# hkust-vgd/scanobjectnn

Hardware: AMD Instinct MI355X
Metric: point-clouds/sec fwd+bwd at B×2048×3, 15-cls (higher is better)
Workload: dtype f32

## Files before the change

### scanobjectnn_amd/csrc/mlp.hip

```cpp
#include <stdlib.h>

#include "common.h"
#include <initializer_list>
#include <type_traits>

#ifndef PCOPS_MLP_PART
#define PCOPS_MLP_PART (-1)
#endif
#define PCOPS_PART(p_) (PCOPS_MLP_PART < 0 || PCOPS_MLP_PART == (p_))
#define PCOPS_HIDDEN __attribute__((visibility("hidden")))

#ifndef PCOPS_BF_RM
#define PCOPS_BF_RM 1
#endif

namespace pcops_mlp {

typedef float f32x16 __attribute__((ext_vector_type(16)));
typedef float f32x4 __attribute__((ext_vector_type(4)));
typedef __bf16 bf16x8 __attribute__((ext_vector_type(8)));

typedef __bf16 bf16x2 __attribute__((ext_vector_type(2)));
typedef float f32x2 __attribute__((ext_vector_type(2)));
__device__ __forceinline__ void split3_pair(float a, float b, bf16x2 &h, bf16x2 &m, bf16x2 &l) {
// ... 4433 lines not shown
        }
    }
}

__global__ __launch_bounds__(256) void pool_top_wsparse_kernel(long long G, int S, int C, int Kp,
                                                               const float *__restrict__ gout,
                                                               const float *__restrict__ ysel,
                                                               const unsigned char *__restrict__ arg,
                                                               const float *__restrict__ sc, const float *__restrict__ sh,
                                                               const float *__restrict__ p,
                                                               const float *__restrict__ Yprev,
                                                               const float *__restrict__ psc, const float *__restrict__ psh,
                                                               float *__restrict__ Ssp, float *__restrict__ cfsum) {
    constexpr int KR = 8, U = 8;
    __shared__ float red[4][64 * KR + 1];
    const int lane = threadIdx.x & 63, wave = threadIdx.x >> 6;
    const int c = blockIdx.x;
    const float scc = sc[c], shc = sh[c], pc = p[c];
    const int kr = (Kp + 63) / 64;
    float asc[KR], ash[KR], acc[KR];
#pragma unroll
    for (int i = 0; i < KR; ++i) {
        const int k = lane + 64 * i;
        asc[i] = (k < Kp && psc) ? psc[k] : 1.f;
        ash[i] = (k < Kp && psc) ? psh[k] : 0.f;
        acc[i] = 0.f;
    }
    float csum = 0.f;
    const long long gq = (G + 3) / 4;
    const long long gend = (wave + 1) * gq < G ? (wave + 1) * gq : G;
    for (long long g0 = wave * gq; g0 < gend; g0 += 64) {
        const long long g = g0 + lane;
        float cf = 0.f;
        int row = 0;
        if (g < gend) {
            const long long e = g * C + c;
            cf = fmaf(ysel[e], scc, shc) > 0.f ? pc * gout[e] : 0.f;
            row = arg[e];
        }
        unsigned long long hits = __ballot(cf != 0.f);
        while (hits) {
            float w[U];
            long long r[U];
#pragma unroll
            for (int u = 0; u < U; ++u) {
                w[u] = 0.f;
                r[u] = 0;
                if (hits) {
                    const int l = __builtin_ctzll(hits);
                    hits &= hits - 1;
                    w[u] = __builtin_bit_cast(float, __builtin_amdgcn_readlane(__builtin_bit_cast(int, cf), l));
                    r[u] = (g0 + l) * S + __builtin_amdgcn_readlane(row, l);
                }
            }
#pragma unroll
            for (int i = 0; i < KR; ++i) {
                if (i >= kr) break;
                const int k = lane + 64 * i;
                float x[U];
#pragma unroll
                for (int u = 0; u < U; ++u) x[u] = (k < Kp) ? Yprev[r[u] * Kp + k] : 0.f;
#pragma unroll
                for (int u = 0; u < U; ++u) {
                    const float xv = psc ? fmaxf(fmaf(x[u], asc[i], ash[i]), 0.f) : x[u];
                    acc[i] = fmaf(w[u], xv, acc[i]);
                }
            }
#pragma unroll
            for (int u = 0; u < U; ++u) csum += w[u];
        }
    }
#pragma unroll
    for (int i = 0; i < KR; ++i) red[wave][lane + 64 * i] = acc[i];
    if (lane == 0) red[wave][64 * KR] = csum;
    __syncthreads();
    for (int k = threadIdx.x; k < Kp; k += 256)
        Ssp[(long long)k * C + c] = (red[0][k] + red[1][k]) + (red[2][k] + red[3][k]);
    if (threadIdx.x == 0)
        cfsum[c] = (red[0][64 * KR] + red[1][64 * KR]) + (red[2][64 * KR] + red[3][64 * KR]);
}

template <int KP>
__global__ __launch_bounds__(1024) void pool_top_addend_rows_kernel(int G, int C, const float *__restrict__ gout,
                                                                    const float *__restrict__ ysel,
                                                                    const unsigned char *__restrict__ arg,
                                                                    const float *__restrict__ sc, const float *__restrict__ sh,
                                                                    const float *__restrict__ p, const float *__restrict__ Wt,
                                                                    const int *__restrict__ block_start,
                                                                    float *__restrict__ addend, int *__restrict__ rowmap) {
    constexpr int LPR = KP / 4, RPP = 256 / LPR;
    constexpr int MAXR = 128, MW = 8;
    extern __shared__ __attribute__((aligned(16))) float lds[];
    float *Ws = lds;
    float *cf = Ws + (size_t)C * KP;
    unsigned *mask = reinterpret_cast<unsigned *>(cf + 4 * 256);
    const int tid = threadIdx.x, sub = tid >> 8, c = tid & 255;
    for (int e = tid; e < C * (KP / 4); e += 1024)
        reinterpret_cast<float4 *>(Ws)[e] = reinterpret_cast<const float4 *>(Wt)[e];
    const float scc = c < C ? sc[c] : 0.f, shc = c < C ? sh[c] : 0.f, pc = c < C ? p[c] : 0.f;
    float *mycf = cf + sub * 256;
    unsigned *mymask = mask + sub * MAXR * MW;
    const int q = c % LPR, rsub = c / LPR;
    float v = 0.f;
    int row = 0, base = 0, nrows = 0;
    auto fetch = [&](long long g) {
        v = 0.f; row = 0; base = 0; nrows = 0;
        if (g < G) {
            const int b0 = block_start[g];
            base = kBlk * b0;
            nrows = kBlk * (block_start[g + 1] - b0);
            nrows = nrows < MAXR ? nrows : MAXR;
            if (c < C) {
                const long long e = g * C + c;
                v = fmaf(ysel[e], scc, shc) > 0.f ? pc * gout[e] : 0.f;
                row = arg[e];
            }
        }
    };
    fetch((long long)blockIdx.x * 4 + sub);
    for (long long g0 = (long long)blockIdx.x * 4; g0 < G; g0 += (long long)gridDim.x * 4) {
        const float cv = v;
        const int crow = row, cbase = base, cnrows = nrows;
        __syncthreads();
        mycf[c] = cv;
#pragma unroll
        for (int i = 0; i < MAXR * MW / 256; ++i) mymask[c + 256 * i] = 0u;
        __syncthreads();
        if (cv != 0.f && crow < cnrows) atomicOr(&mymask[crow * MW + (c >> 5)], 1u << (c & 31));
        __syncthreads();
        fetch(g0 + (long long)gridDim.x * 4 + sub);
        for (int r = rsub; r < cnrows; r += RPP) {
            float4 acc = make_float4(0.f, 0.f, 0.f, 0.f);
            bool any = false;
#pragma unroll
            for (int w = 0; w < MW; ++w) {
                unsigned mm = mymask[r * MW + w];
                any = any || mm != 0u;
                while (mm) {
                    const int ch = 32 * w + __builtin_ctz(mm);
                    mm &= mm - 1u;
                    const float cw = mycf[ch];
                    const float4 wt = *reinterpret_cast<const float4 *>(&Ws[ch * KP + 4 * q]);
                    acc.x = fmaf(cw, wt.x, acc.x); acc.y = fmaf(cw, wt.y, acc.y);
                    acc.z = fmaf(cw, wt.z, acc.z); acc.w = fmaf(cw, wt.w, acc.w);
                }
            }
            const long long ri = (long long)cbase + r;
            if (any) *reinterpret_cast<float4 *>(&addend[ri * KP + 4 * q]) = acc;
            if (q == 0) rowmap[ri] = any ? (int)ri : -1;
        }
    }
}

template <int KP>
__global__ __launch_bounds__(256) void pool_top_wsparse_rows_kernel(int G, int C, int maxr, const float *__restrict__ gout,
                                                                    const float *__restrict__ ysel,
                                                                    const unsigned char *__restrict__ arg,
                                                                    const float *__restrict__ sc, const float *__restrict__ sh,
                                                                    const float *__restrict__ p,
                                                                    const float *__restrict__ Yprev,
                                                                    const float *__restrict__ psc, const float *__restrict__ psh,
                                                                    const int *__restrict__ block_start,
                                                                    float *__restrict__ part, float *__restrict__ part2) {
    constexpr int LD = KP + 1, K4 = KP / 4;
    extern __shared__ __attribute__((aligned(16))) float lds[];
    float *Xs = lds;
    const int tid = threadIdx.x, c = tid;
    const float scc = c < C ? sc[c] : 0.f, shc = c < C ? sh[c] : 0.f, pc = c < C ? p[c] : 0.f;
    const int k4 = tid % K4, r0 = tid / K4;
    const float4 asc = *reinterpret_cast<const float4 *>(psc + 4 * k4), ash = *reinterpret_cast<const float4 *>(psh + 4 * k4);
    float acc[KP];
#pragma unroll
    for (int k = 0; k < KP; ++k) acc[k] = 0.f;
    float csum = 0.f;
    for (int g = blockIdx.x; g < G; g += gridDim.x) {
        const int b0 = block_start[g];
        int nrows = kBlk * (block_start[g + 1] - b0);
        nrows = nrows < maxr ? nrows : maxr;
        const float *src = Yprev + (long long)kBlk * b0 * KP;
        float cfv = 0.f;
        int row = 0;
        if (c < C) {
            const long long e = (long long)g * C + c;
            cfv = fmaf(ysel[e], scc, shc) > 0.f ? pc * gout[e] : 0.f;
            row = arg[e];
            if (row >= nrows) { row = 0; cfv = 0.f; }
        }
        __syncthreads();
        for (int r = r0; r < nrows; r += 256 / K4) {
            float4 x = *reinterpret_cast<const float4 *>(src + (long long)r * KP + 4 * k4);
            x.x = fmaxf(fmaf(x.x, asc.x, ash.x), 0.f); x.y = fmaxf(fmaf(x.y, asc.y, ash.y), 0.f);
            x.z = fmaxf(fmaf(x.z, asc.z, ash.z), 0.f); x.w = fmaxf(fmaf(x.w, asc.w, ash.w), 0.f);
            float *d = &Xs[r * LD + 4 * k4];
            d[0] = x.x; d[1] = x.y; d[2] = x.z; d[3] = x.w;
        }
        __syncthreads();
        const float *xr = &Xs[row * LD];
#pragma unroll
        for (int k = 0; k < KP; ++k) acc[k] = fmaf(cfv, xr[k], acc[k]);
        csum += cfv;
    }
    if (c < C) {
        float *dst = part + (long long)blockIdx.x * KP * C + c;
#pragma unroll
        for (int k = 0; k < KP; ++k) dst[(long long)k * C] = acc[k];
        part2[(long long)blockIdx.x * C + c] = csum;
    }
}

template <int KP, int NR>
__global__ __launch_bounds__(256) void pool_top_wsparse_rows_pipe_kernel(int G, int C, int maxr, const float *__restrict__ gout,
                                                                         const float *__restrict__ ysel,
                                                                         const unsigned char *__restrict__ arg,
                                                                         const float *__restrict__ sc, const float *__restrict__ sh,
                                                                         const float *__restrict__ p,
                                                                         const float *__restrict__ Yprev,
                                                                         const float *__restrict__ psc, const float *__restrict__ psh,
                                                                         const int *__restrict__ block_start,
                                                                         float *__restrict__ part, float *__restrict__ part2) {
    constexpr int LD = KP + 4, K4 = KP / 4, RPP = 256 / K4;
    static_assert(NR * RPP == 64 || NR * RPP == 128, "the launcher sizes an LDS image at 64 or 128 rows (maxr <= NR RPP)");
    extern __shared__ __attribute__((aligned(16))) float lds[];
    const int tid = threadIdx.x, c = tid;
    const float scc = c < C ? sc[c] : 0.f, shc = c < C ? sh[c] : 0.f, pc = c < C ? p[c] : 0.f;
    const int k4 = tid % K4, r0 = tid / K4;
    const float4 asc = *reinterpret_cast<const float4 *>(psc + 4 * k4), ash = *reinterpret_cast<const float4 *>(psh + 4 * k4);
    float acc[KP];
#pragma unroll
    for (int k = 0; k < KP; ++k) acc[k] = 0.f;
    float csum = 0.f;
    const int grid = gridDim.x;
    float4 px[NR];
    float fy = 0.f, fg = 0.f;
    int fa = 0, fn = 0;
    int nb0 = 0, nb1 = 0;
    auto pair = [&](int g) {
        if (g < G) { nb0 = block_start[g]; nb1 = block_start[g + 1]; }
    };
    auto fetch = [&](int g) {
        const int n = g < G ? kBlk * (nb1 - nb0) : 0;
        fn = n < maxr ? n : maxr;
        const __amdgpu_buffer_rsrc_t rx = make_rsrc(Yprev + (long long)kBlk * (g < G ? nb0 : 0) * KP, (long long)fn * KP * 4);
#pragma unroll
        for (int j = 0; j < NR; ++j) px[j] = buf_load4(rx, (unsigned)((r0 + RPP * j) * KP + 4 * k4) * 4u, 0u);
        const long long e = (long long)(g < G ? g : G - 1) * C + (c < C ? c : C - 1);
        fy = ysel[e]; fg = gout[e]; fa = arg[e];
    };
    int g = blockIdx.x;
    pair(g);
    fetch(g);
    pair(g + grid);
    int buf = 0;
    for (; g < G; g += grid) {
        float *Xs = lds + buf * (NR * RPP * LD);
        int t0 = 0, t1 = 0;
        if (g + 2 * grid < G) {
            t0 = block_start[g + 2 * grid];
            t1 = block_start[g + 2 * grid + 1];
        }
#pragma unroll
        for (int j = 0; j < NR; ++j) {
            const int r = r0 + RPP * j;
            float4 x = px[j];
            x.x = fmaxf(fmaf(x.x, asc.x, ash.x), 0.f); x.y = fmaxf(fmaf(x.y, asc.y, ash.y), 0.f);
            x.z = fmaxf(fmaf(x.z, asc.z, ash.z), 0.f); x.w = fmaxf(fmaf(x.w, asc.w, ash.w), 0.f);
            *reinterpret_cast<float4 *>(&Xs[r * LD + 4 * k4]) = x;
        }
        float cfv = fmaf(fy, scc, shc) > 0.f ? pc * fg : 0.f;
        int row = fa;
        if (row >= fn || c >= C) { row = 0; cfv = 0.f; }
        fetch(g + grid);
        nb0 = t0; nb1 = t1;
        __syncthreads();
        const float *xr = &Xs[row * LD];
#pragma unroll
        for (int q = 0; q < K4; ++q) {
            const float4 v = *reinterpret_cast<const float4 *>(xr + 4 * q);
            acc[4 * q] = fmaf(cfv, v.x, acc[4 * q]); acc[4 * q + 1] = fmaf(cfv, v.y, acc[4 * q + 1]);
            acc[4 * q + 2] = fmaf(cfv, v.z, acc[4 * q + 2]); acc[4 * q + 3] = fmaf(cfv, v.w, acc[4 * q + 3]);
        }
        csum += cfv;
        buf ^= 1;
    }
    if (c < C) {
        float *dst = part + (long long)blockIdx.x * KP * C + c;
#pragma unroll
        for (int k = 0; k < KP; ++k) dst[(long long)k * C] = acc[k];
        part2[(long long)blockIdx.x * C + c] = csum;
    }
}

__device__ __forceinline__ void small_gemm_tile(int bx, int by, int M, int K, int N, const float *__restrict__ A, int lda,
                                                         const float *__restrict__ B, int ldb, float *__restrict__ C,
                                                         int ldc, int transA, int transB, const float *__restrict__ bias,
                                                         float *__restrict__ colsum) {
    __shared__ float As[4][32][17], Bs[4][16][33], red[4][32][33], cs[4][2][32];
    const int tid = threadIdx.x, lane = tid & 63, wave = tid >> 6;
    const int m0 = by * 32, n0 = bx * 32;
    const int kchunks = (K + 15) / 16;
    f32x16 acc;
#pragma unroll
    for (int v = 0; v < 16; ++v) acc[v] = 0.f;
    float ra[8], rb[8];
    auto fetch = [&](int ch) {
        const int k0 = ch * 16;
#pragma unroll
// ... 923 lines not shown
    const int groups = bwd_fused_groups(M, K, N, S, gpool != nullptr);
    if (const int rc = bwd_fused_args(a, M >= 1 && K >= 4 && K % 4 == 0 && N >= 1, groups, {xyzw, xyz_stats}, M, K, N, off4,
                                      a_scale, a_shift, G, Y, p, q, t, gpool, argmax, S, W, partial, dW, nullptr, stats_partial))
        return rc;
    a.amode = A_XYZ; a.ldx = 4; a.off4 = off4; a.xw = xyzw; a.xw_ld = K; a.xstats = xyz_stats;
    if (const int rc = set_rows(a, rows)) return rc;
    return bwd_fused_launch(a, true, groups, partial, dW, db, as_stream(stream));
}

int pcops_mlp_wgrad(long long M, int K, int N, const float *X, int ldx, const float *a_scale,
                    const float *a_shift, const float *G, const float *Y, const float *p, const float *q,
                    const float *t, const float *gpool, const unsigned char *argmax, int S,
                    const float *pool_scale, const float *pool_shift, float *partial, float *dW, float *db,
                    pcops_stream_t stream) {
    return pcops_mlp_wgrad_rows(M, K, N, X, ldx, a_scale, a_shift, G, Y, p, q, t, gpool, argmax, S, pool_scale,
                                pool_shift, partial, dW, db, nullptr, stream);
}

int pcops_mlp_wgrad_rows(long long M, int K, int N, const float *X, int ldx, const float *a_scale,
                         const float *a_shift, const float *G, const float *Y, const float *p, const float *q,
                         const float *t, const float *gpool, const unsigned char *argmax, int S,
                         const float *pool_scale, const float *pool_shift, float *partial, float *dW, float *db,
                         const pcops_rows_t *rows, pcops_stream_t stream) {
    PCOPS_REQUIRE_SHAPE(M >= 1 && K >= 1 && N >= 1 && ldx >= K);
    PCOPS_REQUIRE_PTR(X); PCOPS_REQUIRE_PTR(Y); PCOPS_REQUIRE_PTR(p); PCOPS_REQUIRE_PTR(q); PCOPS_REQUIRE_PTR(t);
    PCOPS_REQUIRE_PTR(partial); PCOPS_REQUIRE_PTR(dW);
    if (!gpool) PCOPS_REQUIRE_PTR(G);
    WgradArgs a = {};
    a.M = M; a.K = K; a.N = N;
    a.amode = a_scale ? A_BNRELU : A_PLAIN; a.X = X; a.ldx = ldx; a.asc = a_scale; a.ash = a_shift;
    a.dmode = gpool ? A_DYPOOL : A_DY; a.G = G; a.Y = Y; a.ldy = N; a.p = p; a.q = q; a.t = t;
    a.dsc = pool_scale; a.dsh = pool_shift; a.gpool = gpool; a.argmax = argmax; a.S = S > 0 ? S : 1;
    if (const int rc = set_rows(a, rows)) return rc;
    return wgrad_impl(a, partial, dW, db, as_stream(stream));
}

int pcops_mlp_wgrad_xyz(long long M, int K, int N, const float *off4, const float *xyzw, const float *a_scale,
                        const float *a_shift, const float *G, const float *Y, const float *p, const float *q,
                        const float *t, const float *gpool, const unsigned char *argmax, int S,
                        const float *pool_scale, const float *pool_shift, float *partial, float *dW, float *db,
                        pcops_stream_t stream) {
    return pcops_mlp_wgrad_xyz_rows(M, K, N, off4, xyzw, a_scale, a_shift, G, Y, p, q, t, gpool, argmax, S, pool_scale,
                                    pool_shift, partial, dW, db, nullptr, stream);
}

int pcops_mlp_wgrad_xyz_rows(long long M, int K, int N, const float *off4, const float *xyzw, const float *a_scale,
                             const float *a_shift, const float *G, const float *Y, const float *p, const float *q,
                             const float *t, const float *gpool, const unsigned char *argmax, int S,
                             const float *pool_scale, const float *pool_shift, float *partial, float *dW, float *db,
                             const pcops_rows_t *rows, pcops_stream_t stream) {
    PCOPS_REQUIRE_SHAPE(M >= 1 && K >= 1 && N >= 1);
    PCOPS_REQUIRE_PTR(off4); PCOPS_REQUIRE_PTR(xyzw); PCOPS_REQUIRE_PTR(a_scale); PCOPS_REQUIRE_PTR(a_shift);
    PCOPS_REQUIRE_PTR(Y); PCOPS_REQUIRE_PTR(p); PCOPS_REQUIRE_PTR(q); PCOPS_REQUIRE_PTR(t);
    PCOPS_REQUIRE_PTR(partial); PCOPS_REQUIRE_PTR(dW);
    if (!gpool) PCOPS_REQUIRE_PTR(G);
    if (reinterpret_cast<uintptr_t>(off4) & 15) return PCOPS_ERR_UNSUPPORTED;
    WgradArgs a = {};
    a.M = M; a.K = K; a.N = N;
    a.amode = A_XYZ; a.X = nullptr; a.ldx = K; a.asc = a_scale; a.ash = a_shift;
    a.off4 = off4; a.xw = xyzw; a.xw_ld = K;
    a.dmode = gpool ? A_DYPOOL : A_DY; a.G = G; a.Y = Y; a.ldy = N; a.p = p; a.q = q; a.t = t;
    a.dsc = pool_scale; a.dsh = pool_shift; a.gpool = gpool; a.argmax = argmax; a.S = S > 0 ? S : 1;
    if (const int rc = set_rows(a, rows)) return rc;
    return wgrad_impl(a, partial, dW, db, as_stream(stream));
}

static bool dgrad_top_plan(int M, int Kp, WsPlan *pl) {
    GemmArgs a = {};
    a.M = M; a.K = Kp; a.N = Kp; a.ldx = Kp; a.ldy = Kp;
    return ws_enabled() && Kp % 64 == 0 && Kp <= 512 && ws_plan(a, A_BNRELU, pl);
}

int pcops_mlp_pool_top_supported(int M, int Kp, int N, int S) {
    WsPlan pl;
    if (S < 1 || S > 256 || M % S != 0 || N % 4 != 0 || N > 1024) return 0;
    if (!dgrad_top_plan(M, Kp, &pl)) return 0;
    if (!(wgrad_pc_enabled() && wgrad_pc_shape_ok(M, Kp, Kp, Kp, true))) return 0;
    const long long slots = (long long)(M / S) * (S < N ? S : N);
    return slots * Kp * 4 < (long long)kOOB ? 1 : 0;
}

int pcops_mlp_pool_top_addend(int M, int Kp, int N, int S, const float *gout, const float *ysel,
                            const unsigned char *argmax, const float *pool_scale, const float *pool_shift,
                            const float *p, const float *Wt, float *addend, int *rowmap, pcops_stream_t stream) {
    PCOPS_REQUIRE_SHAPE(M >= 1 && S >= 1 && S <= 256 && M % S == 0 && Kp % 4 == 0 && N >= 1 && N <= 65535);
    PCOPS_REQUIRE_PTR(gout); PCOPS_REQUIRE_PTR(ysel); PCOPS_REQUIRE_PTR(argmax); PCOPS_REQUIRE_PTR(pool_scale);
    PCOPS_REQUIRE_PTR(pool_shift); PCOPS_REQUIRE_PTR(p); PCOPS_REQUIRE_PTR(Wt); PCOPS_REQUIRE_PTR(addend);
    PCOPS_REQUIRE_PTR(rowmap);
    if (reinterpret_cast<uintptr_t>(Wt) & 15 || reinterpret_cast<uintptr_t>(addend) & 15) return PCOPS_ERR_UNSUPPORTED;
    if (N > 1024 || Kp > 512) return PCOPS_ERR_UNSUPPORTED;
    if (M / S <= 512)
        hipLaunchKernelGGL(pool_top_addend_kernel<1024>, dim3(M / S), dim3(1024), 0, as_stream(stream), S, N, Kp,
                           S < N ? S : N, gout, ysel, argmax, pool_scale, pool_shift, p, Wt, addend, rowmap);
    else
        hipLaunchKernelGGL(pool_top_addend_kernel<256>, dim3(M / S), dim3(256), 0, as_stream(stream), S, N, Kp,
                           S < N ? S : N, gout, ysel, argmax, pool_scale, pool_shift, p, Wt, addend, rowmap);
    return pcops_launch_status();
}

int pcops_mlp_gemm_dgrad_top(int M, int Kp, const float *Yprev, const float *prev_scale, const float *prev_shift,
                             const float *Mq, const float *vconst, const float *addend, long long addend_rows,
                             const int *rowmap, float *Gprev, float *stats_partial, pcops_stream_t stream) {
    return pcops_mlp_gemm_dgrad_top_rows(M, Kp, Yprev, prev_scale, prev_shift, Mq, vconst, addend, addend_rows, rowmap, Gprev,
                                         stats_partial, nullptr, stream);
}

static int gram_finish(const GramArgs &g, int gg, float *gram, float *xsum, hipStream_t st) {
    const long long L = (long long)g.K * g.K;
    hipLaunchKernelGGL(sum_partials2_kernel, dim3(cdiv(L, 64) + (xsum ? cdiv(g.K, 64) : 0)), dim3(1024), 0, st, gg, L,
                       g.part, gram, (long long)g.K, g.xpart, xsum);
    hipLaunchKernelGGL(mirror_lower_kernel, dim3(g.K), dim3(256), 0, st, g.K, gram);
    return pcops_launch_status();
}

int pcops_mlp_gram(long long M, int Kp, const float *Yprev, int ldx, const float *a_scale, const float *a_shift,
                   float *partial, float *gram, float *xsum, pcops_stream_t stream) {
    PCOPS_REQUIRE_SHAPE(M >= 1 && Kp >= 1 && ldx >= Kp);
    PCOPS_REQUIRE_PTR(Yprev); PCOPS_REQUIRE_PTR(partial); PCOPS_REQUIRE_PTR(gram);
    PCOPS_REQUIRE_ARG((a_scale == nullptr) == (a_shift == nullptr));
    const int gg = gram_full_groups(M, Kp, ldx, Yprev);
    pcops_note_pipe(0);
    if (gg > 0) {
        hipStream_t st = as_stream(stream);
        GramArgs g = {M, Kp, ldx, Yprev, a_scale, a_shift, partial, partial + (long long)gg * Kp * Kp};
        const int nbk = (Kp + 31) / 32;
        const size_t lds = (size_t)(2 * 32 * nbk + 2 * 32 * (32 * nbk + 4)) * sizeof(float);
        const int rc = gram_full_launch(g, nbk, a_scale != nullptr, gg, lds, st);
        return rc ? rc : gram_finish(g, gg, gram, xsum, st);
    }
    WgradArgs a = {};
    a.M = M; a.K = Kp; a.N = Kp;
    a.amode = a_scale ? A_BNRELU : A_PLAIN; a.X = Yprev; a.ldx = ldx; a.asc = a_scale; a.ash = a_shift;
    a.dmode = A_SELFD; a.G = Yprev; a.Y = Yprev; a.ldy = ldx; a.p = a_scale; a.q = a_scale; a.t = a_shift; a.S = 1;
    return wgrad_impl(a, partial, gram, xsum, as_stream(stream));
}

int pcops_mlp_pool_top_wsparse(int M, int Kp, int N, int S, const float *gout, const float *ysel,
                               const unsigned char *argmax, const float *pool_scale, const float *pool_shift,
                               const float *p, const float *Yprev, const float *prev_scale, const float *prev_shift,
                               float *Ssp, float *cfsum, pcops_stream_t stream) {
    PCOPS_REQUIRE_SHAPE(M >= 1 && S >= 1 && S <= 256 && M % S == 0 && Kp >= 1 && Kp <= 512 && N >= 1);
    PCOPS_REQUIRE_PTR(gout); PCOPS_REQUIRE_PTR(ysel); PCOPS_REQUIRE_PTR(argmax); PCOPS_REQUIRE_PTR(pool_scale);
    PCOPS_REQUIRE_PTR(pool_shift); PCOPS_REQUIRE_PTR(p); PCOPS_REQUIRE_PTR(Yprev);
    PCOPS_REQUIRE_ARG((prev_scale == nullptr) == (prev_shift == nullptr));
    PCOPS_REQUIRE_PTR(Ssp); PCOPS_REQUIRE_PTR(cfsum);
    hipLaunchKernelGGL(pool_top_wsparse_kernel, dim3(N), dim3(256), 0, as_stream(stream), (long long)(M / S), S, N,
                       Kp, gout, ysel, argmax, pool_scale, pool_shift, p, Yprev, prev_scale, prev_shift, Ssp, cfsum);
    return pcops_launch_status();
}


static const int kTopRowsWs = 512;

int pcops_mlp_pool_top_rows_supported(int M, int Kp, int N, int S) {
    if (!pcops_mlp_pool_top_supported(M, Kp, N, S)) return 0;
    if (M < 65536 || S % kBlk != 0 || S > 128 || (Kp != 64 && Kp != 128) || N > 256 || N % 32 != 0) return 0;
    if (!gram_full_groups(M, Kp, Kp, nullptr)) return 0;
    return (long long)M * Kp * 4 < (long long)kOOB ? 1 : 0;
}

unsigned long long pcops_mlp_pool_top_wsparse_rows_partial(int Kp, int N) {
    return (unsigned long long)kTopRowsWs * ((unsigned long long)Kp * N + N);
}

int pcops_mlp_pool_top_addend_rows(int M, int Kp, int N, int S, const float *gout, const float *ysel,
                                   const unsigned char *argmax, const float *pool_scale, const float *pool_shift,
                                   const float *p, const float *Wt, float *addend, int *rowmap, const pcops_rows_t *rows,
                                   pcops_stream_t stream) {
    if (!rows) return pcops_mlp_pool_top_addend(M, Kp, N, S, gout, ysel, argmax, pool_scale, pool_shift, p, Wt, addend, rowmap, stream);
    PCOPS_REQUIRE_SHAPE(M >= 1 && S >= 1 && M % S == 0);
    PCOPS_REQUIRE_PTR(gout); PCOPS_REQUIRE_PTR(ysel); PCOPS_REQUIRE_PTR(argmax); PCOPS_REQUIRE_PTR(pool_scale);
    PCOPS_REQUIRE_PTR(pool_shift); PCOPS_REQUIRE_PTR(p); PCOPS_REQUIRE_PTR(Wt); PCOPS_REQUIRE_PTR(addend);
    PCOPS_REQUIRE_PTR(rowmap);
    { const int rrc = rows_ok(rows); if (rrc) return rrc; }
    if (!pcops_mlp_pool_top_rows_supported(M, Kp, N, S)) return PCOPS_ERR_UNSUPPORTED;
    if (reinterpret_cast<uintptr_t>(Wt) & 15 || reinterpret_cast<uintptr_t>(addend) & 15) return PCOPS_ERR_UNSUPPORTED;
    const int G = M / S;
    const size_t lds = ((size_t)N * Kp + 4 * 256 + 4 * 128 * 8) * sizeof(float);
    const int grid = (G + 3) / 4 < 256 ? (G + 3) / 4 : 256;
    hipStream_t st = as_stream(stream);
    return pcops_dispatch<64, 128>(Kp, PCOPS_ERR_UNSUPPORTED, [&](auto kp_) {
        return pcops_launch_lds(pool_top_addend_rows_kernel<decltype(kp_)::value>, dim3(grid), dim3(1024), lds, 160 * 1024, st, G, N,
                                gout, ysel, argmax, pool_scale, pool_shift, p, Wt, rows->block_start, addend, rowmap);
    });
}

int pcops_mlp_pool_top_wsparse_rows(int M, int Kp, int N, int S, const float *gout, const float *ysel,
                                    const unsigned char *argmax, const float *pool_scale, const float *pool_shift,
                                    const float *p, const float *Yprev, const float *prev_scale, const float *prev_shift,
                                    float *Ssp, float *cfsum, float *partial, const pcops_rows_t *rows,
                                    pcops_stream_t stream) {
    if (!rows) return pcops_mlp_pool_top_wsparse(M, Kp, N, S, gout, ysel, argmax, pool_scale, pool_shift, p, Yprev, prev_scale, prev_shift, Ssp, cfsum, stream);
    PCOPS_REQUIRE_SHAPE(M >= 1 && S >= 1 && M % S == 0);
    PCOPS_REQUIRE_PTR(gout); PCOPS_REQUIRE_PTR(ysel); PCOPS_REQUIRE_PTR(argmax); PCOPS_REQUIRE_PTR(pool_scale);
    PCOPS_REQUIRE_PTR(pool_shift); PCOPS_REQUIRE_PTR(p); PCOPS_REQUIRE_PTR(Yprev); PCOPS_REQUIRE_PTR(prev_scale);
    PCOPS_REQUIRE_PTR(prev_shift); PCOPS_REQUIRE_PTR(Ssp); PCOPS_REQUIRE_PTR(cfsum); PCOPS_REQUIRE_PTR(partial);
    { const int rrc = rows_ok(rows); if (rrc) return rrc; }
    if (!pcops_mlp_pool_top_rows_supported(M, Kp, N, S)) return PCOPS_ERR_UNSUPPORTED;
    if (reinterpret_cast<uintptr_t>(Yprev) & 15 || reinterpret_cast<uintptr_t>(prev_scale) & 15 ||
        reinterpret_cast<uintptr_t>(prev_shift) & 15)
        return PCOPS_ERR_UNSUPPORTED;
    const int G = M / S;
    const int grid = G < kTopRowsWs ? G : kTopRowsWs;
    const size_t lds = (size_t)S * (Kp + 1) * sizeof(float);
    float *part2 = partial + (long long)kTopRowsWs * Kp * N;
    hipStream_t st = as_stream(stream);
    const int img_rows = S <= 64 ? 64 : 128;
    if (S > img_rows) return PCOPS_ERR_UNSUPPORTED;
    const size_t lds_pipe = (size_t)2 * img_rows * (Kp + 4) * sizeof(float);
    const bool piped = pcops_get_option(PCOPS_OPT_POOL_TOP_ROWS_PIPELINED) != 0;
    const int rc = pcops_dispatch<64, 128>(Kp, PCOPS_ERR_UNSUPPORTED, [&](auto kp_) {
        constexpr int KP = decltype(kp_)::value;
        auto kern = !piped ? pool_top_wsparse_rows_kernel<KP>
                  : S <= 64 ? pool_top_wsparse_rows_pipe_kernel<KP, KP / 16> : pool_top_wsparse_rows_pipe_kernel<KP, KP / 8>;
        return pcops_launch_lds(kern, dim3(grid), dim3(256), piped ? lds_pipe : lds, 160 * 1024, st, G, N, S, gout, ysel, argmax,
                                pool_scale, pool_shift, p, Yprev, prev_scale, prev_shift, rows->block_start, partial, part2);
    });
    if (rc) return rc;
    const long long L = (long long)Kp * N;
    hipLaunchKernelGGL(sum_partials2_kernel, dim3(cdiv(L, 64) + cdiv(N, 64)), dim3(1024), 0, st, grid, L, partial, Ssp,
                       (long long)N, part2, cfsum);
    return pcops_launch_status();
}

int pcops_mlp_gemm_dgrad_top_rows(int M, int Kp, const float *Yprev, const float *prev_scale, const float *prev_shift,
                                  const float *Mq, const float *vconst, const float *addend, long long addend_rows,
                                  const int *rowmap, float *Gprev, float *stats_partial, const pcops_rows_t *rows,
                                  pcops_stream_t stream) {
    PCOPS_REQUIRE_SHAPE(M >= 1 && Kp >= 1);
    PCOPS_REQUIRE_PTR(Yprev); PCOPS_REQUIRE_PTR(Mq);
    PCOPS_REQUIRE_PTR(vconst); PCOPS_REQUIRE_PTR(addend); PCOPS_REQUIRE_PTR(rowmap); PCOPS_REQUIRE_PTR(Gprev);
    PCOPS_REQUIRE_ARG((prev_scale == nullptr) == (prev_shift == nullptr));
    WsPlan pl;
    if (!dgrad_top_plan(M, Kp, &pl)) return PCOPS_ERR_UNSUPPORTED;
    GemmArgs a = {};
    a.M = M; a.K = Kp; a.N = Kp; a.X = Yprev; a.ldx = Kp; a.v0 = prev_scale; a.v1 = prev_shift;
    a.W = Mq; a.Y = Gprev; a.ldy = Kp; a.Yprev = Yprev; a.msc = prev_scale; a.msh = prev_shift;
    a.stats = stats_partial; a.addend = addend; a.rowmap = rowmap; a.add_ld = Kp; a.vconst = vconst;
    a.add_bytes = addend_rows * Kp * 4;
    if (addend_rows < 1 || a.add_bytes >= (long long)kOOB) return PCOPS_ERR_UNSUPPORTED;
    if (const int rc = set_rows(a, rows)) return rc;
    if (!prev_scale) {
        a.stats = nullptr;
        return launch_gemm_ws_only<A_PLAIN, E_PLAINA>(a, as_stream(stream));
    }
    return launch_gemm_ws_only<A_BNRELU, E_MASKA>(a, as_stream(stream));
}

int pcops_mlp_gram_rows(long long M, int Kp, const float *Yprev, int ldx, const float *a_scale, const float *a_shift,
                        float *partial, float *gram, float *xsum, const pcops_rows_t *rows, pcops_stream_t stream) {
    if (!rows) return pcops_mlp_gram(M, Kp, Yprev, ldx, a_scale, a_shift, partial, gram, xsum, stream);
    PCOPS_REQUIRE_SHAPE(M >= 1 && Kp >= 1 && ldx >= Kp);
    PCOPS_REQUIRE_PTR(Yprev); PCOPS_REQUIRE_PTR(partial); PCOPS_REQUIRE_PTR(gram); PCOPS_REQUIRE_PTR(a_scale);
    PCOPS_REQUIRE_PTR(a_shift);
    { const int rrc = rows_ok(rows); if (rrc) return rrc; }
    const int gg = gram_full_groups(M, Kp, ldx, Yprev);
    if (gg <= 0 || (Kp != 64 && Kp != 128)) return PCOPS_ERR_UNSUPPORTED;
    pcops_note_pipe(0);
    hipStream_t st = as_stream(stream);
    GramArgs g = {M, Kp, ldx, Yprev, a_scale, a_shift, partial, partial + (long long)gg * Kp * Kp,
                  static_cast<const RowBlock *>(rows->blocks), rows->rows};
    const int nbk = Kp / 32;
    const size_t lds = (size_t)(2 * 32 * nbk + 2 * 32 * (32 * nbk + 4)) * sizeof(float);
    const bool bf3 = Kp == 128 && pcops_get_option(PCOPS_OPT_GRAM_SPLIT_BF16) != 0;
    const int rc = bf3 ? gram_rows_bf3_launch(g, gg, st) : gram_full_rows_launch(g, nbk, gg, lds, st);
    if (rc) return rc;
    if (bf3) pcops_note_pipe(1);
    return gram_finish(g, gg, gram, xsum, st);
}

int pcops_mlp_dy_apply(long long M, int N, const float *G, const float *Y, const float *p, const float *q, const float *t,
                       float *out, pcops_stream_t stream) {
    PCOPS_REQUIRE_SHAPE(M >= 0 && N >= 4 && N % 4 == 0);
    if (M == 0) return PCOPS_OK;
    PCOPS_REQUIRE_PTR(G); PCOPS_REQUIRE_PTR(Y); PCOPS_REQUIRE_PTR(p); PCOPS_REQUIRE_PTR(q); PCOPS_REQUIRE_PTR(t); PCOPS_REQUIRE_PTR(out);
    PCOPS_REQUIRE_ARG(((uintptr_t)G | (uintptr_t)Y | (uintptr_t)p | (uintptr_t)q | (uintptr_t)t | (uintptr_t)out) % 16 == 0);
    const long long total4 = M * (N / 4);
    const unsigned grid = (unsigned)(cdiv(total4, 256) < 8192 ? cdiv(total4, 256) : 8192);
    hipLaunchKernelGGL(dy_apply_kernel, dim3(grid), dim3(256), 0, as_stream(stream), total4, N / 4,
                       reinterpret_cast<const float4 *>(G), reinterpret_cast<const float4 *>(Y),
                       reinterpret_cast<const float4 *>(p), reinterpret_cast<const float4 *>(q),
                       reinterpret_cast<const float4 *>(t), reinterpret_cast<float4 *>(out));
    return pcops_launch_status();
}

int pcops_mlp_pool_top_prep(int Kp, int N, const float *W, const float *b, const float *q, const float *t, float *Wt,
                            float *Wq, float *u, float *v, pcops_stream_t stream) {
    PCOPS_REQUIRE_SHAPE(Kp >= 1 && N >= 1);
    PCOPS_REQUIRE_PTR(W); PCOPS_REQUIRE_PTR(b); PCOPS_REQUIRE_PTR(q); PCOPS_REQUIRE_PTR(t);
    PCOPS_REQUIRE_PTR(Wt); PCOPS_REQUIRE_PTR(Wq); PCOPS_REQUIRE_PTR(u);
    const int gx = (N + 31) / 32;
    hipLaunchKernelGGL(pool_top_prep_kernel, dim3(gx, (Kp + 31) / 32 + (v ? ((Kp + 7) / 8 + gx - 1) / gx : 0)), dim3(256), 0,
                       as_stream(stream), Kp, N, W, b, q, t, Wt, Wq, u, v);
    return pcops_launch_status();
}

int pcops_mlp_pool_top_finish(int Kp, int N, long long M, float *dW, const float *Ssp, const float *xsum, const float *u,
                              const float *cfsum, const float *q, const float *W, const float *b, const float *t,
                              float *db, pcops_stream_t stream) {
    PCOPS_REQUIRE_SHAPE(Kp >= 1 && N >= 1 && M >= 1);
    PCOPS_REQUIRE_PTR(dW); PCOPS_REQUIRE_PTR(Ssp); PCOPS_REQUIRE_PTR(xsum); PCOPS_REQUIRE_PTR(u); PCOPS_REQUIRE_PTR(cfsum);
    PCOPS_REQUIRE_PTR(q); PCOPS_REQUIRE_PTR(W); PCOPS_REQUIRE_PTR(b); PCOPS_REQUIRE_PTR(t); PCOPS_REQUIRE_PTR(db);
    hipLaunchKernelGGL(pool_top_finish_kernel, dim3((N + 255) / 256, 8 + (Kp + 7) / 8), dim3(256), 0, as_stream(stream), Kp, N,
                       (float)M, dW, Ssp, xsum, u, cfsum, q, W, b, t, db);
    return pcops_launch_status();
}

int pcops_small_gemm(int M, int K, int N, const float *A, int lda, const float *B, int ldb, float *C, int ldc,
                     pcops_stream_t stream) {
    return pcops_small_gemm_ex(M, K, N, A, lda, 0, B, ldb, 0, nullptr, C, ldc, stream);
}

int pcops_small_gemm_ex(int M, int K, int N, const float *A, int lda, int transA, const float *B, int ldb, int transB,
                        const float *bias, float *C, int ldc, pcops_stream_t stream) {
    return pcops_small_gemm_colsum(M, K, N, A, lda, transA, B, ldb, transB, bias, C, ldc, nullptr, stream);
}

int pcops_small_gemm_colsum(int M, int K, int N, const float *A, int lda, int transA, const float *B, int ldb, int transB,
                            const float *bias, float *C, int ldc, float *colsum, pcops_stream_t stream) {
    PCOPS_REQUIRE_SHAPE(M >= 1 && K >= 1 && N >= 1 && lda >= (transA ? M : K) && ldb >= (transB ? K : N) && ldc >= N);
    PCOPS_REQUIRE_PTR(A); PCOPS_REQUIRE_PTR(B); PCOPS_REQUIRE_PTR(C);
    pcops_note_pipe(0);
    hipLaunchKernelGGL(small_gemm_kernel, dim3((N + 31) / 32, (M + 31) / 32), dim3(256), 0, as_stream(stream), M, K, N, A,
                       lda, B, ldb, C, ldc, transA ? 1 : 0, transB ? 1 : 0, bias, colsum);
    return pcops_launch_status();
}

int pcops_small_gemm_pair(const pcops_gemm_problem_t *p, pcops_stream_t stream) {
    PCOPS_REQUIRE_PTR(p);
    SgProblem q[2];
    int tiles[2], gx[2];
    for (int i = 0; i < 2; ++i) {
        const pcops_gemm_problem_t &a = p[i];
        PCOPS_REQUIRE_SHAPE(a.M >= 1 && a.K >= 1 && a.N >= 1 && a.lda >= (a.transA ? a.M : a.K) && a.ldb >= (a.transB ? a.K : a.N) &&
                            a.ldc >= a.N);
// ... 32 lines not shown
```

Measured before the change: 26030.

## Add software-pipelined wave-per-group pool-top addend rows kernel behind option

Adds a new kernel that assigns one wavefront per group and uses ballot/ff1 scalar bit scanning to find the channels hitting each row. It prefetches the next group's inputs and block starts while the current group is processed, and overlaps weight-row LDS loads for row r+1 with the accumulation for row r. The goal is to hide global-load latency and avoid the per-row mask arrays of the old kernel. It is gated by an option, so whether it runs depends on that option's default. The wrapper's shape check is also relaxed, dropping the M and full-group requirements for the addend path.

```diff
diff --git a/scanobjectnn_amd/csrc/mlp.hip b/scanobjectnn_amd/csrc/mlp.hip
--- a/scanobjectnn_amd/csrc/mlp.hip
+++ b/scanobjectnn_amd/csrc/mlp.hip
@@ -4609,6 +4609,150 @@
     }
 }
 
+template <int KP, int MAXR>
+__global__ __launch_bounds__(1024) void pool_top_addend_rows_pipe_kernel(int G, int C, const float *__restrict__ gout,
+                                                                         const float *__restrict__ ysel,
+                                                                         const unsigned char *__restrict__ arg,
+                                                                         const float *__restrict__ sc, const float *__restrict__ sh,
+                                                                         const float *__restrict__ p, const float *__restrict__ Wt,
+                                                                         const int *__restrict__ block_start,
+                                                                         float *__restrict__ addend, int *__restrict__ rowmap) {
+    constexpr int VEC = KP / 64, NW = 4;
+    static_assert(VEC == 1 || VEC == 2, "a row is one or two floats per lane");
+    static_assert(MAXR == 64 || MAXR == 128, "lane l answers for the rows l and l + 64 of a group");
+    typedef float rowv_t __attribute__((ext_vector_type(VEC)));
+    extern __shared__ __attribute__((aligned(16))) float lds[];
+    float *Ws = lds + KP;
+    const int tid = threadIdx.x, lane = tid & 63;
+    const int wave = __builtin_amdgcn_readfirstlane(tid >> 6);
+    for (int e = tid; e < C * (KP / 4); e += 1024)
+        reinterpret_cast<float4 *>(Ws)[e] = reinterpret_cast<const float4 *>(Wt)[e];
+    if (tid < KP) lds[tid] = 0.f;
+    float scc[NW], shc[NW], pc[NW];
+#pragma unroll
+    for (int k = 0; k < NW; ++k) {
+        const int c = lane + 64 * k;
+        scc[k] = c < C ? sc[c] : 0.f; shc[k] = c < C ? sh[c] : 0.f; pc[k] = c < C ? p[c] : 0.f;
+    }
+    __syncthreads();
+    float fy[NW], fg[NW];
+    int fa[NW], fbase = 0, fn = 0;
+    int nb0 = 0, nb1 = 0;
+    auto pair = [&](long long g) {
+        if (g < G) { nb0 = block_start[g]; nb1 = block_start[g + 1]; }
+    };
+    auto fetch = [&](long long g) {
+        fbase = 0; fn = 0;
+        if (g < G) {
+            fbase = kBlk * nb0;
+            fn = kBlk * (nb1 - nb0);
+            fn = fn < MAXR ? fn : MAXR;
+        }
+#pragma unroll
+        for (int k = 0; k < NW; ++k) {
+            const int c = lane + 64 * k;
+            fy[k] = 0.f; fg[k] = 0.f; fa[k] = 0;
+            if (g < G && c < C) {
+                const long long e = g * C + c;
+                fy[k] = ysel[e]; fg[k] = gout[e]; fa[k] = arg[e];
+            }
+        }
+    };
+    const long long stride = (long long)gridDim.x * 16;
+    long long g = (long long)blockIdx.x * 16 + wave;
+    auto ff1 = [](unsigned long long m) {
+        int l;
+        asm("s_ff1_i32_b64 %0, %1" : "=s"(l) : "s"(m));
+        return l;
+    };
+    auto bit_clear = [](unsigned long long &m, int l) { asm("s_bitset0_b64 %0, %1" : "+s"(m) : "s"(l)); };
+    auto bit_set = [](unsigned long long &m, int l) { asm("s_bitset1_b64 %0, %1" : "+s"(m) : "s"(l)); };
+    int wbase[NW];
+#pragma unroll
+    for (int k = 0; k < NW; ++k) wbase[k] = ((64 * k - 1) * KP + VEC * lane) * 4;
+    auto wrow = [&](int k, int l) {
+        return *reinterpret_cast<const rowv_t *>(reinterpret_cast<const char *>(Ws) + (wbase[k] + (l + 1) * (KP * 4)));
+    };
+    pair(g);
+    fetch(g);
+    pair(g + stride);
+    for (; g < G; g += stride) {
+        int t0 = 0, t1 = 0;
+        if (g + 2 * stride < G) {
+            t0 = block_start[g + 2 * stride];
+            t1 = block_start[g + 2 * stride + 1];
+        }
+        float cfv[NW];
+        int rowv[NW];
+#pragma unroll
+        for (int k = 0; k < NW; ++k) {
+            cfv[k] = fmaf(fy[k], scc[k], shc[k]) > 0.f ? pc[k] * fg[k] : 0.f;
+            rowv[k] = (cfv[k] != 0.f && fa[k] < fn) ? fa[k] : -1;
+        }
+        const int base = fbase, nrows = fn;
+        fetch(g + stride);
+        nb0 = t0; nb1 = t1;
+        asm volatile("" ::"s"(nb0), "s"(nb1));
+        struct Set {
+            rowv_t w[NW];
+            float cf[NW];
+            unsigned long long m[NW];
+            int l[NW];
+        };
+        auto coef = [&](int k, int l) {
+            return __builtin_bit_cast(float, __builtin_amdgcn_readlane(__builtin_bit_cast(int, cfv[k]), l));
+        };
+        auto issue = [&](int r, Set &s) {
+#pragma unroll
+            for (int k = 0; k < NW; ++k) {
+                s.m[k] = __ballot(rowv[k] == r);
+                s.l[k] = ff1(s.m[k]);
+                s.cf[k] = coef(k, s.l[k]);
+                s.w[k] = wrow(k, s.l[k]);
+            }
+        };
+        unsigned long long anylo = 0ull, anyhi = 0ull;
+        char *const dst = reinterpret_cast<char *>(addend) + VEC * 4 * lane;
+        auto finish = [&](int r, const Set &s) {
+            rowv_t acc = 0.f;
+            bool any = false;
+#pragma unroll
+            for (int k = 0; k < NW; ++k) {
+                if (s.l[k] >= 0) {
+                    asm volatile("" ::: "memory");
+                    any = true;
+#pragma unroll
+                    for (int i = 0; i < VEC; ++i) acc[i] = fmaf(s.cf[k], s.w[k][i], acc[i]);
+                    unsigned long long mm = s.m[k];
+                    bit_clear(mm, s.l[k]);
+                    while (mm) {
+                        const int l = ff1(mm);
+                        bit_clear(mm, l);
+                        const float cw = coef(k, l);
+                        const rowv_t wt = wrow(k, l);
+#pragma unroll
+                        for (int i = 0; i < VEC; ++i) acc[i] = fmaf(cw, wt[i], acc[i]);
+                    }
+                }
+            }
+            if (any) {
+                *reinterpret_cast<rowv_t *>(dst + (unsigned)(base + r) * (unsigned)(KP * 4)) = acc;
+                if (MAXR == 64 || r < 64) bit_set(anylo, r); else bit_set(anyhi, r - 64);
+            }
+        };
+        Set A, B;
+        issue(0, A);
+        for (int r = 0; r < nrows; r += 2) {
+            issue(r + 1, B);
+            finish(r, A);
+            issue(r + 2, A);
+            if (r + 1 < nrows) finish(r + 1, B);
+        }
+        if (lane < nrows) rowmap[(long long)base + lane] = (anylo >> lane) & 1ull ? base + lane : -1;
+        if (MAXR > 64 && lane + 64 < nrows) rowmap[(long long)base + lane + 64] = (anyhi >> lane) & 1ull ? base + lane + 64 : -1;
+    }
+}
+
 template <int KP>
 __global__ __launch_bounds__(256) void pool_top_wsparse_rows_kernel(int G, int C, int maxr, const float *__restrict__ gout,
                                                                     const float *__restrict__ ysel,
@@ -5838,11 +5982,15 @@
 
 static const int kTopRowsWs = 512;
 
+static bool addend_rows_shape_ok(int M, int Kp, int N, int S) {
+    return S % kBlk == 0 && S <= 128 && (Kp == 64 || Kp == 128) && N <= 256 && N % 32 == 0 &&
+           (long long)M * Kp * 4 < (long long)kOOB;
+}
+
 int pcops_mlp_pool_top_rows_supported(int M, int Kp, int N, int S) {
     if (!pcops_mlp_pool_top_supported(M, Kp, N, S)) return 0;
-    if (M < 65536 || S % kBlk != 0 || S > 128 || (Kp != 64 && Kp != 128) || N > 256 || N % 32 != 0) return 0;
-    if (!gram_full_groups(M, Kp, Kp, nullptr)) return 0;
-    return (long long)M * Kp * 4 < (long long)kOOB ? 1 : 0;
+    if (M < 65536 || !addend_rows_shape_ok(M, Kp, N, S)) return 0;
+    return gram_full_groups(M, Kp, Kp, nullptr) ? 1 : 0;
 }
 
 unsigned long long pcops_mlp_pool_top_wsparse_rows_partial(int Kp, int N) {
@@ -5859,14 +6007,20 @@
     PCOPS_REQUIRE_PTR(pool_shift); PCOPS_REQUIRE_PTR(p); PCOPS_REQUIRE_PTR(Wt); PCOPS_REQUIRE_PTR(addend);
     PCOPS_REQUIRE_PTR(rowmap);
     { const int rrc = rows_ok(rows); if (rrc) return rrc; }
-    if (!pcops_mlp_pool_top_rows_supported(M, Kp, N, S)) return PCOPS_ERR_UNSUPPORTED;
+    if (!addend_rows_shape_ok(M, Kp, N, S)) return PCOPS_ERR_UNSUPPORTED;
     if (reinterpret_cast<uintptr_t>(Wt) & 15 || reinterpret_cast<uintptr_t>(addend) & 15) return PCOPS_ERR_UNSUPPORTED;
     const int G = M / S;
     const size_t lds = ((size_t)N * Kp + 4 * 256 + 4 * 128 * 8) * sizeof(float);
     const int grid = (G + 3) / 4 < 256 ? (G + 3) / 4 : 256;
     hipStream_t st = as_stream(stream);
+    const bool piped = pcops_get_option(PCOPS_OPT_POOL_TOP_ROWS_PIPELINED) != 0;
+    const size_t lds_pipe = (size_t)(N + 1) * Kp * sizeof(float);
+    const int grid_pipe = (G + 15) / 16 < 256 ? (G + 15) / 16 : 256;
     return pcops_dispatch<64, 128>(Kp, PCOPS_ERR_UNSUPPORTED, [&](auto kp_) {
-        return pcops_launch_lds(pool_top_addend_rows_kernel<decltype(kp_)::value>, dim3(grid), dim3(1024), lds, 160 * 1024, st, G, N,
+        constexpr int KP = decltype(kp_)::value;
+        auto kern = !piped ? pool_top_addend_rows_kernel<KP>
+                  : S <= 64 ? pool_top_addend_rows_pipe_kernel<KP, 64> : pool_top_addend_rows_pipe_kernel<KP, 128>;
+        return pcops_launch_lds(kern, dim3(piped ? grid_pipe : grid), dim3(1024), piped ? lds_pipe : lds, 160 * 1024, st, G, N,
                                 gout, ysel, argmax, pool_scale, pool_shift, p, Wt, rows->block_start, addend, rowmap);
     });
 }
```

New measurement: 26390 (median of 6 runs). +1.4%, better.
